# FlowEternal/multitask-hydranet

Hardware: AMD Instinct MI355X
Metric: images/sec (fwd+bwd) HydraNet @ default res, 1/2/4/8 MI355X; CPU-ref same run (higher is better)
Workload: dtype bf16; 1 GPU; full HydraNet (backbone + BiFPN + seg/det/lane heads + multitask loss), big cfg, fwd+loss+bwd; batch_per_gpu=16, global_batch=16, resolution=3x512x1024, parallelism=dp1, hipgraph=True

## Files before the change

include/hydranet_hip.h:

```cpp
#ifndef HYDRANET_HIP_H
#define HYDRANET_HIP_H

#ifdef __cplusplus
extern "C" {
#endif

typedef struct ihipStream_t* hipStream_t;


int hn_gconv_pack_diag(const float* w, void* wk, void* wd, int C, hipStream_t stream);
int hn_pack_weight(const float* w, void* wp, void* wt, int Cout, int Cin, int taps, hipStream_t stream);
int hn_pack_weight_ex(const float* w, void* wp, void* wt, int Cout, int Cin_total, int ci0, int Cin, int taps, int phase, const float* bias,
                      float* b_eff, hipStream_t stream);
int hn_phase_fold(const float* dw_eff, const float* dw1, const float* db_eff, float* dw, float* db, int K, int C0, int C1, hipStream_t stream);
int hn_pack_weights_batched(const long* jobs, int njobs, long total_blocks, const int* block_job, hipStream_t stream);
int hn_pack_small_batched(const long* jobs, const int* block_job, long total_blocks, hipStream_t stream);

int hn_conv_gemm_nt(const void* x0, const void* x1, int mode, int n_img, int H, int W, int C0, int C1, int ld0, int ld1, int up, long M,
                    const void* w, int Nout, int KP, int taps, const float* bias, int act, void* out, int out_f32, int ldc, long rpi,
                    long img_stride, float* psum, float* psq, hipStream_t stream);
int hn_nt_stat_rows(long M, int Nout);
int hn_nt_stat_tile(long M, int Nout);
int hn_conv_gemm_nt_stream(const void* x, int ld0, long M, int C0, const void* w, int Nout, int KP, const float* bias, int act, void* out,
                           int ldc, float* psum, float* psq, int wg_limit, hipStream_t stream);
// ... 6 lines not shown
                        int ldc, const float* coef, int nlev, const long* rows, hipStream_t stream);
int hn_conv_gemm_nt_lvlout(const void* x0, int ld0, long M, int C0, const void* w, int Nout, int KP, const float* bias, int act, float* out,
                           int ldc, long img_stride, int n_img, int nlev, const int* H, const int* W, int row_align, hipStream_t stream);

int hn_conv_gemm_nt_ex(const void* x0, const void* x1, int mode, int n_img, int H, int W, int C0, int C1, int ld0, int ld1, int up, long M,
                       const void* w, int Nout, int KP, int taps, const float* bias, int act, void* out, int out_f32, int ldc, long rpi,
                       long img_stride, float* psum, float* psq, const float* xscale, const float* xshift, const float* xgate, long xhw,
                       int xact, const void* addend, int ld_add, int add_mode, hipStream_t stream);
int hn_conv_gemm_nt_stat(const void* x0, const void* x1, int mode, int n_img, int H, int W, int C0, int C1, int ld0, int ld1, int up, long M,
                         const void* w, int Nout, int KP, int taps, const float* bias, int act, void* out, int out_f32, int ldc, long rpi,
                         long img_stride, float* psum, float* psq, const void* addend, int ld_add, int add_mode, int emode, const void* ez,
                         int ld_ez, const float* ecoef, hipStream_t stream);
int hn_conv_gemm_nt_stat3(const void* x0, int ld0, long M, int C0, const void* w, int Nout, int KP, void* out, int ldc, float* psum, float* psq,
                          const void* addend, int ld_add, const void* ez, int ld_ez, const void* ey, int ld_ey, const float* ecoef,
                          hipStream_t stream);
int hn_wgrad_plan(int mode, int n_img, int H, int W, long M, int Nout, int KP, int taps, int* splits, long* rows_per_split, long* ws_bytes);
int hn_conv_gemm_tn(const void* x0, const void* x1, int mode, int n_img, int H, int W, int C0, int C1, int ld0, int ld1, int up, long M,
                    const void* dz, int ldz, int Nout, int KP, int taps, float* workspace, float* dw, hipStream_t stream);


int hn_stem_fwd(const float* x, const float* w, void* z, void* patches, int N, int H, int W, hipStream_t stream);

int hn_gconv_pack(const float* w, void* wk, void* wd, int C, int flip, hipStream_t stream);
int hn_gconv_fwd(const void* in, int ldi, const void* wk, void* out, int ldo, int N, int Hi, int Wi, int C, int stride, hipStream_t stream);
int hn_gconv_dgrad_s2(const void* dz, int ldz, const void* wd, void* dx, int ldx, int N, int Hi, int Wi, int C, hipStream_t stream);
long hn_wgrad_chunks(long pixels, long items);
int hn_gconv_wgrad(const void* x, int ldx, const void* dz, int ldz, float* part, int N, int Hi, int Wi, int C, int stride,
                   hipStream_t stream);

int hn_dw_pack(const float* w, void* wk, void* wkf, int C, hipStream_t stream);
int hn_dwconv_fwd(const void* in, int ldi, const void* wk, void* out, int ldo, int N, int H, int W, int C, hipStream_t stream);
int hn_dwconv_fwd_levels(const void* in, int ldi, const void* wk, void* out, int ldo, int N, int C, int nlev, const int* H, const int* W,
                         int row_align, int accumulate, hipStream_t stream);
long hn_dwconv_wgrad_blocks(long strips, int C);
int hn_dwconv_wgrad(const void* x, int ldx, const void* dz, int ldz, float* part, int N, int H, int W, int C, hipStream_t stream);
int hn_dwconv_wgrad_levels(const void* x, int ldx, const void* dz, int ldz, float* part, int N, int C, int nlev, const int* H, const int* W,
                           int row_align, hipStream_t stream);
long hn_dwconv_bwd_blocks(long strips, int C);
long hn_dwconv_bwd_blocks_levels(int N, int C, int nlev, const int* H, const int* W);
int hn_dwconv_bwd_levels(const void* dz, int ldz, const void* x, int ldx, const void* wf, void* dx, int lddx, float* part, int N, int C,
                         int nlev, const int* H, const int* W, int row_align, int accumulate, hipStream_t stream);

int hn_maxpool_fwd(const void* in, int ldi, void* out, int ldo, int N, int H, int W, int C, int mode, hipStream_t stream);
int hn_maxpool_bwd(const void* in, int ldi, const void* dout, int ldd, void* dx, int ldx, const float* wscale, int N, int H, int W, int C,
                   int mode, hipStream_t stream);
int hn_maxpool_bwd2(const void* in, int ldi, const void* dout, int ldd, void* dx, int ldx, const float* wscale, void* arg_ws, int N, int H,
                    int W, int C, int mode, int accumulate, hipStream_t stream);

int hn_up2_fwd(const void* in, int ldi, void* out, int ldo, int N, int H, int W, int C, hipStream_t stream);
int hn_sum2x2(const void* g, int ldg, void* out, int ldo, const float* wscale, int N, int H, int W, int C, int accumulate, hipStream_t stream);

int hn_fuse_dweights(const float* pw, int blocks, const float* praw, int nw, float eps, float* dp, hipStream_t stream);
int hn_fuse_fwd(const void* const* in, const int* ld, const int* mode, const float* w, void* out, int ldo, int N, int H, int W, int C,
                hipStream_t stream);
int hn_fuse_fwd_raw(const void* const* in, const int* ld, const int* mode, const float* praw, int nw, float eps, float* wn, void* out, int ldo,
                    int N, int H, int W, int C, hipStream_t stream);
int hn_fuse_bwd_blocks(int N, int H, int W, int C);
int hn_fuse_bwd(const void* const* in, const int* ld, const int* mode, const float* w, const void* dout, int ldd, void* g, int ldg,
                void* const* din, const int* ldin, const int* acc, float* pw, int N, int H, int W, int C, hipStream_t stream);
int hn_fuse_bwd_arg(const void* const* in, const int* ld, const int* mode, const float* w, const void* dout, int ldd, void* g, int ldg,
                    void* const* din, const int* ldin, const int* acc, float* pw, void* const* arg_out, int N, int H, int W, int C,
                    hipStream_t stream);
int hn_maxpool_bwd_from_arg(const void* arg, const void* dout, int ldd, void* dx, int ldx, const float* wscale, int N, int H, int W, int C,
                            int mode, int accumulate, hipStream_t stream);

long hn_fold_ring_rows(int H, int W);
// ... 359 lines not shown
```

multitask_hydranet_amd/csrc/hn_stencil.hip:

```cpp
#include "hn_common.h"

__global__ __launch_bounds__(256) void stem_fwd_kernel(const float* x, const float* w, bf16* z, bf16* patches, int N, int H, int W) {
    const int bidx = xcd_remap(blockIdx.x, gridDim.x);
    __shared__ float sw[27][32];
    for (int i = threadIdx.x; i < 27 * 32; i += 256) {
        const int co = i & 31, t = i >> 5;
        sw[t][co] = w[co * 27 + t];
    }
    __syncthreads();
    const int Ho = H >> 1, Wo = W >> 1, Wp = (Wo + 1) >> 1;
    const long total = (long)N * Ho * Wp;
    const long idx = (long)bidx * 256 + threadIdx.x;
    if (idx >= total) return;
    const int ox = (int)(idx % Wp) * 2;
    const long t1 = idx / Wp;
    const int oy = (int)(t1 % Ho);
    const long n = t1 / Ho;
    const bool two = ox + 1 < Wo;
    float acc[2][32];
#pragma unroll
    for (int c = 0; c < 32; ++c) { acc[0][c] = 0.f; acc[1][c] = 0.f; }
    __shared__ __attribute__((aligned(16))) bf16 sp[2][256][36];
    bf16* prow = patches ? sp[0][threadIdx.x] : nullptr;
    constexpr int PH = 256 * 36;
// ... 830 lines not shown
                    bf16x4 v;
                    if (accumulate) {
                        const bf16x4 prev = ld4(dst);
#pragma unroll
                        for (int k = 0; k < 4; ++k) v[k] = f2bf(da[k] + bf2f(prev[k]));
                    } else {
#pragma unroll
                        for (int k = 0; k < 4; ++k) v[k] = f2bf(da[k]);
                    }
                    *reinterpret_cast<bf16x4*>(dst) = v;
                }
            }
        }
    }
    __syncthreads();
    float* red = reinterpret_cast<float*>(smem);
    if (active) {
#pragma unroll
        for (int tq = 0; tq < 9; ++tq)
#pragma unroll
            for (int k = 0; k < 4; ++k) red[(colh * C4 + cq) * 37 + tq * 4 + k] = acc[tq][k];
    }
    __syncthreads();
    float* dst = part + (long)bidx * C * 9;
    for (int o = tid; o < C4 * 36; o += 256) {
        const int g = o / 36, v = o - g * 36;
        float sum = 0.f;
#pragma unroll
        for (int c2 = 0; c2 < 8; ++c2) sum += red[(c2 * C4 + g) * 37 + v];
        dst[(long)(g * 4 + (v & 3)) * 9 + (v >> 2)] = sum;
    }
}

__global__ void dw_pack_kernel(const float* w, bf16* wk, bf16* wkf, int C) {
    const int idx = blockIdx.x * blockDim.x + threadIdx.x;
    if (idx >= 9 * C) return;
    const int c = idx % C, tap = idx / C;
    const bf16 v = f2bf(w[c * 9 + tap]);
    wk[idx] = v;
    if (wkf) wkf[(8 - tap) * C + c] = v;
}

__device__ __forceinline__ void pool_window(const bf16* in, int ldi, long n, int H, int W, int oy, int ox, int c, int mode, float* best,
                                            int* arg) {
#pragma unroll
    for (int k = 0; k < 8; ++k) { best[k] = -INFINITY; arg[k] = -1; }
    const int off = mode ? -1 : 0;
#pragma unroll
    for (int ky = 0; ky < 3; ++ky)
#pragma unroll
        for (int kx = 0; kx < 3; ++kx) {
            const int iy = 2 * oy + ky + off, ix = 2 * ox + kx + off;
            const bool inside = iy >= 0 && iy < H && ix >= 0 && ix < W;
            if (!inside && mode) continue;
            bf16x8 v = inside ? ld8(in + ((n * H + iy) * (long)W + ix) * ldi + c) : zero8();
#pragma unroll
            for (int k = 0; k < 8; ++k) {
                const float f = bf2f(v[k]);
                if (f > best[k]) { best[k] = f; arg[k] = inside ? ky * 3 + kx : 9; }
            }
        }
}

__global__ __launch_bounds__(256) void maxpool_fwd_kernel(const bf16* in, int ldi, bf16* out, int ldo, int N, int H, int W, int C,
                                                          int mode) {
    const int bidx = xcd_remap(blockIdx.x, gridDim.x);
// ... 284 lines not shown
        const int yq = (int)(t % Hq);
        const long n = t / Hq;
        float qsum[8];
#pragma unroll
        for (int k = 0; k < 8; ++k) qsum[k] = 0.f;
        for (int sub = 0; sub < (quads ? 4 : 1); ++sub) {
        const int x = quads ? 2 * xq + (sub & 1) : xq, y = quads ? 2 * yq + (sub >> 1) : yq;
        float v[3][8], pre[8];
#pragma unroll
        for (int k = 0; k < 8; ++k) pre[k] = 0.f;
#pragma unroll
        for (int i = 0; i < 3; ++i) {
            if (!p.mode[i]) continue;
            if (p.mode[i] == 3 && q.arg[i]) {
                int a[8];
                pool_window(p.in[i], p.ld[i], n, 2 * p.H, 2 * p.W, y, x, cg * 8, 0, v[i], a);
                unsigned long long packed = 0ull;
#pragma unroll
                for (int k = 0; k < 8; ++k) packed |= (unsigned long long)(a[k] & 0xff) << (8 * k);
                *reinterpret_cast<unsigned long long*>(q.arg[i] + ((n * p.H + y) * (long)p.W + x) * p.C + cg * 8) = packed;
            } else {
                fuse_gather(p, i, n, y, x, cg * 8, v[i]);
            }
            const float wi = p.w[i];
#pragma unroll
            for (int k = 0; k < 8; ++k) pre[k] = fmaf(wi, v[i][k], pre[k]);
        }
        const long orow = (n * p.H + y) * (long)p.W + x;
        const bf16x8 d = ld8(q.dout + orow * q.ldd + cg * 8);
        float gg[8];
        bf16x8 go;
#pragma unroll
        for (int k = 0; k < 8; ++k) { gg[k] = bf2f(d[k]) * act_bwd(pre[k], HN_ACT_SWISH); go[k] = f2bf(gg[k]); qsum[k] += bf2f(go[k]); }
        st8(q.g + orow * q.ldg + cg * 8, go);
#pragma unroll
        for (int i = 0; i < 3; ++i) {
            if (!p.mode[i]) continue;
#pragma unroll
            for (int k = 0; k < 8; ++k) dw[i] = fmaf(gg[k], v[i][k], dw[i]);
            if (p.mode[i] == 1 && q.din[i]) {
                const float wi = p.w[i];
                bf16* dst = q.din[i] + orow * q.ldin[i] + cg * 8;
                bf16x8 o;
                if (q.acc[i]) {
                    const bf16x8 prev = ld8(dst);
#pragma unroll
                    for (int k = 0; k < 8; ++k) o[k] = f2bf(fmaf(wi, gg[k], bf2f(prev[k])));
                } else {
#pragma unroll
                    for (int k = 0; k < 8; ++k) o[k] = f2bf(wi * gg[k]);
                }
                st8(dst, o);
            }
        }
        }
        if (quads) {
            const float ws = p.w[up_i];
            bf16* dst = q.din[up_i] + ((n * Hq + yq) * (long)Wq + xq) * q.ldin[up_i] + cg * 8;
            bf16x8 o;
            if (q.acc[up_i]) {
                const bf16x8 prev = ld8(dst);
#pragma unroll
                for (int k = 0; k < 8; ++k) o[k] = f2bf(fmaf(qsum[k], ws, bf2f(prev[k])));
            } else {
#pragma unroll
                for (int k = 0; k < 8; ++k) o[k] = f2bf(qsum[k] * ws);
            }
// ... 35 lines not shown
        const int yq = (int)(t % Hq);
        const long n = t / Hq;
        const long orow0 = (n * p.H + 2 * yq) * (long)p.W + 2 * xq, lrow = (n * Hq + yq) * (long)Wq + xq;
        bf16x8 rd[4], ra[4], rprev[4], rup, rprev_up;
#pragma unroll
        for (int s = 0; s < 4; ++s) rd[s] = ld8(q.dout + (orow0 + (s >> 1) * p.W + (s & 1)) * q.ldd + cg * 8);
#pragma unroll
        for (int s = 0; s < 4; ++s) ra[s] = ld8(ina + (orow0 + (s >> 1) * p.W + (s & 1)) * lda + cg * 8);
        rup = ld8(inb + lrow * ldb + cg * 8);
        if (acca) {
#pragma unroll
            for (int s = 0; s < 4; ++s) rprev[s] = ld8(da + (orow0 + (s >> 1) * p.W + (s & 1)) * ldda + cg * 8);
        }
        bf16* dup = db + lrow * lddb + cg * 8;
        if (accb) rprev_up = ld8(dup);
        float qsum[8], vb[8];
#pragma unroll
        for (int k = 0; k < 8; ++k) { qsum[k] = 0.f; vb[k] = bf2f(rup[k]); }
#pragma unroll
        for (int s = 0; s < 4; ++s) {
            const long orow = orow0 + (s >> 1) * p.W + (s & 1);
            float gg[8];
            bf16x8 go;
#pragma unroll
            for (int k = 0; k < 8; ++k) {
                const float va = bf2f(ra[s][k]);
                const float pre = a_first ? fmaf(wb, vb[k], fmaf(wa, va, 0.f)) : fmaf(wa, va, fmaf(wb, vb[k], 0.f));
                gg[k] = bf2f(rd[s][k]) * act_bwd(pre, HN_ACT_SWISH);
                go[k] = f2bf(gg[k]);
                qsum[k] += bf2f(go[k]);
                dwa = fmaf(gg[k], va, dwa);
                dwb = fmaf(gg[k], vb[k], dwb);
            }
            st8(q.g + orow * q.ldg + cg * 8, go);
            if (da) {
                bf16x8 o;
                if (acca) {
#pragma unroll
                    for (int k = 0; k < 8; ++k) o[k] = f2bf(fmaf(wa, gg[k], bf2f(rprev[s][k])));
                } else {
#pragma unroll
                    for (int k = 0; k < 8; ++k) o[k] = f2bf(wa * gg[k]);
                }
                st8(da + orow * ldda + cg * 8, o);
            }
        }
        bf16x8 o;
        if (accb) {
#pragma unroll
            for (int k = 0; k < 8; ++k) o[k] = f2bf(fmaf(qsum[k], wb, bf2f(rprev_up[k])));
        } else {
#pragma unroll
            for (int k = 0; k < 8; ++k) o[k] = f2bf(qsum[k] * wb);
        }
        st8(dup, o);
    }
    __shared__ float red[4][3];
    const int lane = threadIdx.x & 63, wave = threadIdx.x >> 6;
    float dw[3] = {0.f, 0.f, 0.f};
#pragma unroll
    for (int i = 0; i < 3; ++i) dw[i] = i == ia ? dwa : (i == ib ? dwb : 0.f);
#pragma unroll
    for (int i = 0; i < 3; ++i) {
        const float sm = wave_sum(dw[i]);
        if (lane == 0) red[wave][i] = sm;
    }
    __syncthreads();
// ... 241 lines not shown
    HN_CHECK_ARG(x && dz && part && (C & 7) == 0 && C <= 2048 && ((ldx | ldz) & 7) == 0);
    L.work_off[0] = 0;
    for (int l = 0; l < L.n; ++l) L.work_off[l + 1] = L.work_off[l] + (long)N * L.H[l] * ((L.W[l] + 3) >> 2);
    const long strips = L.work_off[L.n];
    const int lanes = 256 / (C >> 3);
    const long blocks = hn_dwconv_wgrad_blocks(strips, C);
    const int spl = (int)((strips + blocks * lanes - 1) / (blocks * lanes));
    hipLaunchKernelGGL(dwconv_wgrad_kernel, dim3(blocks), dim3(256), 0, st, (const bf16*)x, ldx, (const bf16*)dz, ldz, part, N, C, spl, L);
    HN_LAUNCH_CHECK();
}
extern "C" int hn_dwconv_wgrad(const void* x, int ldx, const void* dz, int ldz, float* part, int N, int H, int W, int C, hipStream_t st) {
    Levels L;
    const int rc = fill_levels(L, N, 1, &H, &W);
    return rc != HN_OK ? rc : dwconv_wgrad_launch(x, ldx, dz, ldz, part, N, C, L, st);
}
extern "C" int hn_dwconv_wgrad_levels(const void* x, int ldx, const void* dz, int ldz, float* part, int N, int C, int nlev, const int* H,
                                      const int* W, int row_align, hipStream_t st) {
    Levels L;
    const int rc = fill_levels(L, N, nlev, H, W, row_align);
    return rc != HN_OK ? rc : dwconv_wgrad_launch(x, ldx, dz, ldz, part, N, C, L, st);
}

static long dwconv_bwd_strip_blocks(long strips, int C) {
    const int lanes = 256 / (C >> 2);
    const long tb = g_hn_knob[7] > 0 ? g_hn_knob[7] : 768;
    long spl = (strips + (tb - 1) * lanes) / (tb * lanes);
    if (spl < 2) spl = 2;
    return (strips + spl * lanes - 1) / (spl * lanes);
}
extern "C" long hn_dwconv_bwd_blocks(long strips, int C) { return dwconv_bwd_strip_blocks(strips, C); }
static size_t dwconv_bwd_tiled_lds(int C8) {
    return (size_t)((((DWT_TH + 2) * 18 * C8 + 63) >> 6) + ((DWT_TH * 16 * C8 + 63) >> 6)) * 1024;
}
static bool dwconv_bwd_tiled_plan(int N, int C, const Levels& L, DwTiles& T, int& tpw, long& blocks) {
    T.tile_off[0] = 0;
    for (int l = 0; l < L.n; ++l) {
        T.ty[l] = (L.H[l] + DWT_TH - 1) / DWT_TH;
        T.tx[l] = (L.W[l] + 15) >> 4;
        T.tile_off[l + 1] = T.tile_off[l] + (long)N * T.ty[l] * T.tx[l];
    }
    const long total = T.tile_off[L.n];
    const int C8 = C >> 3;
    const size_t lds = dwconv_bwd_tiled_lds(C8);
#ifdef HN_NO_DW_TILED
    return false;
#endif
    if (g_hn_knob[7] < 0 || C8 > 16 || lds > 80 * 1024 || total < 512) return false;
    tpw = (int)((total + 511) / 512);
    blocks = (total + tpw - 1) / tpw;
    return true;
}
extern "C" long hn_dwconv_bwd_blocks_levels(int N, int C, int nlev, const int* H, const int* W) {
    Levels L;
    if (fill_levels(L, N, nlev, H, W) != HN_OK || (C & 7) || C < 8) return -1;
    DwTiles T;
    int tpw = 0;
    long blocks = 0;
    if (dwconv_bwd_tiled_plan(N, C, L, T, tpw, blocks)) return blocks;
    long strips = 0;
    for (int l = 0; l < nlev; ++l) strips += (long)N * H[l] * ((W[l] + 3) >> 2);
    return dwconv_bwd_strip_blocks(strips, C);
}
extern "C" int hn_dwconv_bwd_levels(const void* dz, int ldz, const void* x, int ldx, const void* wf, void* dx, int lddx, float* part, int N, int C,
                                    int nlev, const int* H, const int* W, int row_align, int accumulate, hipStream_t st) {
    Levels L;
    const int rc = fill_levels(L, N, nlev, H, W, row_align);
    if (rc != HN_OK) return rc;
    HN_CHECK_ARG(dz && x && part && (!dx || wf) && (C & 7) == 0 && C >= 8 && C <= 1024 && ((ldz | ldx) & 7) == 0 && (!dx || (lddx & 7) == 0));
    long pad_items = 0;
    if (dx && !accumulate)
        for (int l = 0; l < L.n; ++l) pad_items += (L.row_off[l + 1] - L.row_off[l] - (long)N * L.H[l] * L.W[l]) * (C >> 3);
    DwTiles T;
    int tpw = 0;
    long tblocks = 0;
    if (dwconv_bwd_tiled_plan(N, C, L, T, tpw, tblocks)) {
        const int C8 = C >> 3;
        const size_t lds = dwconv_bwd_tiled_lds(C8);
        if (lds > 64 * 1024) {
            static std::atomic<unsigned long long> optin_t{0};
            if (!lds_optin(optin_t, {(const void*)dwconv_bwd_tiled_kernel<true>, (const void*)dwconv_bwd_tiled_kernel<false>})) return HN_ERR_LAUNCH;
        }
        L.work_off[0] = 0;
        if (dx)
            hipLaunchKernelGGL(dwconv_bwd_tiled_kernel<true>, dim3((unsigned)(tblocks + cdiv(pad_items, 256))), dim3(256), lds, st, (const bf16*)dz,
                               ldz, (const bf16*)x, ldx, (const bf16*)wf, (bf16*)dx, lddx, part, N, C, tpw, (int)tblocks, L, T, accumulate);
        else
            hipLaunchKernelGGL(dwconv_bwd_tiled_kernel<false>, dim3((unsigned)tblocks), dim3(256), lds, st, (const bf16*)dz, ldz, (const bf16*)x, ldx,
                               (const bf16*)wf, (bf16*)dx, lddx, part, N, C, tpw, (int)tblocks, L, T, accumulate);
        HN_LAUNCH_CHECK();
    }
    L.work_off[0] = 0;
    for (int l = 0; l < L.n; ++l) L.work_off[l + 1] = L.work_off[l] + (long)N * L.H[l] * ((L.W[l] + 3) >> 2);
    const long strips = L.work_off[L.n];
    const int lanes = 256 / (C >> 2);
    const long blocks = dwconv_bwd_strip_blocks(strips, C);
    const int spl = (int)((strips + blocks * lanes - 1) / (blocks * lanes));
    const size_t lds = (256 * 37 + 9 * (size_t)C) * sizeof(float);
    if (lds > 64 * 1024) {
        static std::atomic<unsigned long long> optin{0};
        if (!lds_optin(optin, {(const void*)dwconv_bwd_kernel})) return HN_ERR_LAUNCH;
    }
    hipLaunchKernelGGL(dwconv_bwd_kernel, dim3((unsigned)(blocks + cdiv(pad_items, 256))), dim3(256), lds, st, (const bf16*)dz, ldz, (const bf16*)x,
                       ldx, (const bf16*)wf, (bf16*)dx, lddx, part, N, C, spl, blocks, L, accumulate);
    HN_LAUNCH_CHECK();
}

extern "C" int hn_maxpool_fwd(const void* in, int ldi, void* out, int ldo, int N, int H, int W, int C, int mode, hipStream_t st) {
    HN_CHECK_ARG(in && out && (C & 7) == 0 && ((ldi | ldo) & 7) == 0 && !(H & 1) && !(W & 1) && (mode == 0 || mode == 1));
    hipLaunchKernelGGL(maxpool_fwd_kernel, dim3(ew_grid((long)N * (H >> 1) * (W >> 1) * (C >> 3))), dim3(256), 0, st, (const bf16*)in, ldi,
                       (bf16*)out, ldo, N, H, W, C, mode);
    HN_LAUNCH_CHECK();
}
extern "C" int hn_maxpool_bwd(const void* in, int ldi, const void* dout, int ldd, void* dx, int ldx, const float* wscale, int N, int H,
                              int W, int C, int mode, hipStream_t st) {
    HN_CHECK_ARG(in && dout && dx && (C & 7) == 0 && ((ldi | ldd | ldx) & 7) == 0 && !(H & 1) && !(W & 1));
    hipLaunchKernelGGL(maxpool_bwd_kernel, dim3(ew_grid((long)N * H * W * (C >> 3))), dim3(256), 0, st, (const bf16*)in, ldi,
                       (const bf16*)dout, ldd, (bf16*)dx, ldx, wscale, N, H, W, C, mode);
    HN_LAUNCH_CHECK();
}
extern "C" int hn_maxpool_bwd2(const void* in, int ldi, const void* dout, int ldd, void* dx, int ldx, const float* wscale, void* arg_ws,
                               int N, int H, int W, int C, int mode, int accumulate, hipStream_t st) {
    HN_CHECK_ARG(in && dout && dx && arg_ws && (C & 7) == 0 && ((ldi | ldd | ldx) & 7) == 0 && !(H & 1) && !(W & 1));
    hipLaunchKernelGGL(maxpool_arg_kernel, dim3(ew_grid((long)N * (H >> 1) * (W >> 1) * (C >> 3))), dim3(256), 0, st, (const bf16*)in, ldi,
                       (unsigned char*)arg_ws, N, H, W, C, mode);
    hipLaunchKernelGGL(maxpool_bwd_arg_kernel, dim3(ew_grid((long)N * H * W * (C >> 3))), dim3(256), 0, st, (const unsigned char*)arg_ws,
                       (const bf16*)dout, ldd, (bf16*)dx, ldx, wscale, N, H, W, C, mode, accumulate);
    HN_LAUNCH_CHECK();
}
extern "C" int hn_maxpool_bwd_from_arg(const void* arg, const void* dout, int ldd, void* dx, int ldx, const float* wscale, int N, int H, int W,
                                       int C, int mode, int accumulate, hipStream_t st) {
    HN_CHECK_ARG(arg && dout && dx && (C & 7) == 0 && ((ldd | ldx) & 7) == 0 && !(H & 1) && !(W & 1));
    hipLaunchKernelGGL(maxpool_bwd_arg_kernel, dim3(ew_grid((long)N * H * W * (C >> 3))), dim3(256), 0, st, (const unsigned char*)arg,
                       (const bf16*)dout, ldd, (bf16*)dx, ldx, wscale, N, H, W, C, mode, accumulate);
    HN_LAUNCH_CHECK();
}
extern "C" int hn_up2_fwd(const void* in, int ldi, void* out, int ldo, int N, int H, int W, int C, hipStream_t st) {
    HN_CHECK_ARG(in && out && (C & 7) == 0 && ((ldi | ldo) & 7) == 0);
    hipLaunchKernelGGL(up2_fwd_kernel, dim3(ew_grid((long)N * 4 * H * W * (C >> 3))), dim3(256), 0, st, (const bf16*)in, ldi, (bf16*)out, ldo,
                       N, H, W, C);
// ... 13 lines not shown
    for (int i = 0; i < 3; ++i) {
        f.in[i] = (const bf16*)in[i]; f.ld[i] = ld[i]; f.mode[i] = mode[i];
        HN_CHECK_ARG(mode[i] >= 0 && mode[i] <= 3 && (mode[i] == 0 || (in[i] && (ld[i] & 7) == 0)));
        HN_CHECK_ARG(mode[i] != 2 || (!(H & 1) && !(W & 1)));
    }
    f.w = w; f.out = (bf16*)out; f.ldo = ldo; f.N = N; f.H = H; f.W = W; f.C = C;
    f.praw = nullptr; f.nw = 0; f.eps = 0.f; f.wn = nullptr;
    return HN_OK;
}
extern "C" int hn_fuse_fwd(const void* const* in, const int* ld, const int* mode, const float* w, void* out, int ldo, int N, int H, int W,
                           int C, hipStream_t st) {
    Fuse f;
    HN_CHECK_ARG(out);
    const int rc = fill_fuse(f, in, ld, mode, w, out, ldo, N, H, W, C);
    if (rc) return rc;
    hipLaunchKernelGGL(fuse_fwd_kernel, dim3(ew_grid((long)N * H * W * (C >> 3))), dim3(256), 0, st, f);
    HN_LAUNCH_CHECK();
}
extern "C" int hn_fuse_fwd_raw(const void* const* in, const int* ld, const int* mode, const float* praw, int nw, float eps, float* wn,
                               void* out, int ldo, int N, int H, int W, int C, hipStream_t st) {
    Fuse f;
    HN_CHECK_ARG(out && praw && wn && nw >= 1 && nw <= 3);
    const int rc = fill_fuse(f, in, ld, mode, nullptr, out, ldo, N, H, W, C);
    if (rc) return rc;
    f.praw = praw; f.nw = nw; f.eps = eps; f.wn = wn;
    hipLaunchKernelGGL(fuse_fwd_kernel, dim3(ew_grid((long)N * H * W * (C >> 3))), dim3(256), 0, st, f);
    HN_LAUNCH_CHECK();
}
extern "C" int hn_fuse_bwd_blocks(int N, int H, int W, int C) {
    long b = ((long)N * H * W * (C >> 3) + 255) / 256;
    if (b > 1024) b = 1024;
    return (int)(b < 1 ? 1 : b);
}
extern "C" int hn_fuse_bwd(const void* const* in, const int* ld, const int* mode, const float* w, const void* dout, int ldd, void* g,
                           int ldg, void* const* din, const int* ldin, const int* acc, float* pw, int N, int H, int W, int C,
                           hipStream_t st) {
    FuseBwd q;
    HN_CHECK_ARG(dout && g && pw && din && ldin && ((ldd | ldg) & 7) == 0);
    const int rc = fill_fuse(q.f, in, ld, mode, w, nullptr, 8, N, H, W, C);
    if (rc) return rc;
    q.dout = (const bf16*)dout; q.ldd = ldd; q.g = (bf16*)g; q.ldg = ldg; q.pw = pw;
    for (int i = 0; i < 3; ++i) { q.din[i] = (bf16*)din[i]; q.ldin[i] = ldin[i]; q.acc[i] = acc ? acc[i] : 0; q.arg[i] = nullptr; }
    int n_id = 0, n_up = 0, n_pool = 0, up_dst = 0;
    for (int i = 0; i < 3; ++i) { n_id += mode[i] == 1; n_up += mode[i] == 2; n_pool += mode[i] == 3; up_dst += mode[i] == 2 && q.din[i]; }
    if (n_id == 1 && n_up == 1 && up_dst == 1 && n_pool == 0 && !(H & 1) && !(W & 1))
        hipLaunchKernelGGL(fuse_bwd_quads_kernel, dim3(hn_fuse_bwd_blocks(N, H, W, C)), dim3(256), 0, st, q);
    else
        hipLaunchKernelGGL(fuse_bwd_kernel, dim3(hn_fuse_bwd_blocks(N, H, W, C)), dim3(256), 0, st, q);
    HN_LAUNCH_CHECK();
}
extern "C" int hn_fuse_bwd_arg(const void* const* in, const int* ld, const int* mode, const float* w, const void* dout, int ldd, void* g,
                               int ldg, void* const* din, const int* ldin, const int* acc, float* pw, void* const* arg_out, int N, int H,
                               int W, int C, hipStream_t st) {
    FuseBwd q;
    HN_CHECK_ARG(dout && g && pw && din && ldin && arg_out && ((ldd | ldg) & 7) == 0);
    const int rc = fill_fuse(q.f, in, ld, mode, w, nullptr, 8, N, H, W, C);
    if (rc) return rc;
    q.dout = (const bf16*)dout; q.ldd = ldd; q.g = (bf16*)g; q.ldg = ldg; q.pw = pw;
    for (int i = 0; i < 3; ++i) {
        q.din[i] = (bf16*)din[i]; q.ldin[i] = ldin[i]; q.acc[i] = acc ? acc[i] : 0;
        q.arg[i] = mode[i] == 3 ? (unsigned char*)arg_out[i] : nullptr;
    }
    int n_id = 0, n_up = 0, n_pool = 0, up_dst = 0;
    for (int i = 0; i < 3; ++i) { n_id += mode[i] == 1; n_up += mode[i] == 2; n_pool += mode[i] == 3; up_dst += mode[i] == 2 && q.din[i]; }
    if (n_id == 1 && n_up == 1 && up_dst == 1 && n_pool == 0 && !(H & 1) && !(W & 1))
        hipLaunchKernelGGL(fuse_bwd_quads_kernel, dim3(hn_fuse_bwd_blocks(N, H, W, C)), dim3(256), 0, st, q);
    else
        hipLaunchKernelGGL(fuse_bwd_kernel, dim3(hn_fuse_bwd_blocks(N, H, W, C)), dim3(256), 0, st, q);
    HN_LAUNCH_CHECK();
}

extern "C" int hn_seg_fold(const void* dvp, int ldv, int c0, void* out, int ldo, const void* yprev, int ldy, int N, int H, int W, int C,
                           int up, hipStream_t st) {
    HN_CHECK_ARG(dvp && out && (C & 7) == 0 && (c0 & 7) == 0 && ((ldv | ldo) & 7) == 0 && H >= 4 && W >= 4 && up >= 0 && up <= 2);
    HN_CHECK_ARG(!yprev || (ldy & 7) == 0);
    const int clamp = up == 2;
    if (clamp) up = 0;
    hipLaunchKernelGGL(seg_fold_kernel, dim3(ew_grid((long)N * (H >> up) * (W >> up) * (C >> 3))), dim3(256), 0, st, (const bf16*)dvp, ldv, c0,
                       (bf16*)out, ldo, (const bf16*)yprev, ldy, N, H, W, C, up, clamp);
    HN_LAUNCH_CHECK();
}

extern "C" int hn_space_to_depth(const float* dy, void* out, int ldo, int N, int h, int w, int k, hipStream_t st) {
    HN_CHECK_ARG(dy && out && N > 0 && h > 0 && w > 0 && k > 0 && ldo >= 4 * k && (ldo & 7) == 0);
    hipLaunchKernelGGL(space_to_depth_kernel, dim3(ew_grid((long)N * h * w * ldo)), dim3(256), 0, st, dy, (bf16*)out, ldo, N, h, w, k);
    HN_LAUNCH_CHECK();
}

extern "C" int hn_space_to_depth_blocks(int N, int h, int w, int k) { return ew_grid((long)N * h * w * 4 * (k >> 3)); }
extern "C" int hn_space_to_depth_bf16(const void* in, int ldi, void* out, int N, int h, int w, int k, float* psum, hipStream_t st) {
// ... 93 lines not shown
```

multitask_hydranet_amd/ops/heads.py:

```python
from __future__ import annotations

import ctypes
import os
from typing import Optional, Sequence, Tuple

import torch

from .._lib import lib, policy
from .core import *
from .backbone import *
from .neck import *
from .seg import *


class HeadOut(torch.autograd.Function):

    @staticmethod
    def forward(ctx, dw_weight, pw_weight, bias, k, act, *feats):
        n = feats[0].shape[0]
        cout, cin = pw_weight.shape[0], pw_weight.shape[1]
        wp, wt = pack_conv_weight(pw_weight)
        rows_total = sum(f.shape[1] * f.shape[2] for f in feats)
        rep = cout // k
        out = torch.empty((n, rows_total * rep, k), device=feats[0].device, dtype=F32)
# ... 113 lines not shown
        d6 = new_act(n, h // 2, w // 2, c, dout.device)
        lib().call("hn_sum2x2", ptr(dout[..., 3 * c:]), ld(dout), ptr(d6), ld(d6), None, n, h // 2, w // 2, c, 0)
        return d3, d4, d5, d6



def packed_rows(geom):
    n, hs, ws = geom
    return sum(_pad_rows(n * h * w) for h, w in zip(hs, ws))


def has_pad_rows(geom):
    n, hs, ws = geom
    return any((n * h * w) % LEVEL_ALIGN for h, w in zip(hs, ws))


def _ptr_array(tensors):
    return (ctypes.c_void_p * len(tensors))(*[t.data_ptr() if t is not None else None for t in tensors])


def level_views(packed, geom):
    n, hs, ws = geom
    out, off = [], 0
    for h, w in zip(hs, ws):
        m = n * h * w
        out.append(packed[0, 0, off:off + m].view(n, h, w, packed.shape[3]))
        off += _pad_rows(m)
    return out


def k_dwconv_levels(x, wk, geom, into=None):
    nl, H, W, _, _ = _geom_arrays(geom)
    out = torch.empty_like(x) if into is None else into
    lib().call("hn_dwconv_fwd_levels", ptr(x), ld(x), ptr(wk), ptr(out), ld(out), geom[0], x.shape[3], nl, ctypes.addressof(H),
               ctypes.addressof(W), LEVEL_ALIGN, 0 if into is None else 1)
    return out


def k_dwconv_wgrad_levels(x, dz, geom):
    nl, H, W, _, _ = _geom_arrays(geom)
    c = x.shape[3]
    chunks = lib().query("hn_dwconv_wgrad_blocks", sum(geom[0] * hh * ((ww + 3) // 4) for hh, ww in zip(geom[1], geom[2])), c)
    part = torch.empty((chunks, c * 9), device=x.device, dtype=F32)
    lib().call("hn_dwconv_wgrad_levels", ptr(x), ld(x), ptr(dz), ld(dz), ptr(part), geom[0], c, nl, ctypes.addressof(H), ctypes.addressof(W),
               LEVEL_ALIGN)
    return k_rows_reduce(part, 1, chunks, c * 9).view(c, 1, 3, 3)


class PackLevels(torch.autograd.Function):

    @staticmethod
    def forward(ctx, *feats):
        n, c = feats[0].shape[0], feats[0].shape[3]
        geom = (n, tuple(f.shape[1] for f in feats), tuple(f.shape[2] for f in feats))
        total = packed_rows(geom)
        out = torch.empty((1, 1, total, c), device=feats[0].device, dtype=BF16)
        if PACK_LEVELS_ONE and all(f.stride(3) == 1 and f.stride(1) == f.shape[2] * f.stride(2) and f.stride(0) == f.shape[1] * f.stride(1)
                                   for f in feats):
            nl, H, W, _, _ = _geom_arrays(geom)
            lds = (ctypes.c_int * nl)(*[ld(f) for f in feats])
            srcs = _ptr_array(feats)
            lib().call("hn_pack_levels", ctypes.addressof(srcs), ctypes.addressof(lds), ptr(out), ld(out), n, c, nl,
                       ctypes.addressof(H), ctypes.addressof(W), LEVEL_ALIGN)
        else:
            for v, f in zip(level_views(out, geom), feats):
                k_eltwise(2, f, alpha=1.0, out=v)
# ... 174 lines not shown
```

multitask_hydranet_amd/ops/neck.py:

```python
from __future__ import annotations

import ctypes
import os
from typing import Optional, Sequence, Tuple

import torch

from .._lib import lib, policy
from .core import *
from .backbone import *


def k_dwconv(x, wk, out=None):
    n, h, w, c = x.shape
    if out is None:
        out = new_act(n, h, w, c, x.device)
    lib().call("hn_dwconv_fwd", ptr(x), ld(x), ptr(wk), ptr(out), ld(out), n, h, w, c)
    return out


def k_dwconv_wgrad(x, dz):
    n, h, w, c = x.shape
    chunks = lib().query("hn_dwconv_wgrad_blocks", n * h * ((w + 3) // 4), c)
    part = torch.empty((chunks, c * 9), device=x.device, dtype=F32)
    lib().call("hn_dwconv_wgrad", ptr(x), ld(x), ptr(dz), ld(dz), ptr(part), n, h, w, c)
    return k_rows_reduce(part, 1, chunks, c * 9).view(c, 1, 3, 3)


def k_dwconv_bwd(dz, x, wf, geom=None, want_dx=True, into=None, queue=None, weight=None):
    c = x.shape[3]
    if geom is None:
        n, h, w, _ = x.shape
        H, W, nl, align = (ctypes.c_int * 1)(h), (ctypes.c_int * 1)(w), 1, 1
    else:
        nl, H, W, _, _ = _geom_arrays(geom)
        n, align = geom[0], LEVEL_ALIGN
    blocks = lib().query("hn_dwconv_bwd_blocks_levels", n, c, nl, ctypes.addressof(H), ctypes.addressof(W))
    part = torch.empty((blocks, c * 9), device=x.device, dtype=F32)
    dx = None
    if want_dx:
        dx = torch.empty_like(dz) if into is None else into
    lib().call("hn_dwconv_bwd_levels", ptr(dz), ld(dz), ptr(x), ld(x), ptr(wf), ptr(dx), ld(dx) if dx is not None else 0, ptr(part), n, c, nl,
               ctypes.addressof(H), ctypes.addressof(W), align, 0 if into is None else 1)
    if queue is not None:
        queue.add_rows(weight, part, blocks, c * 9, (c, 1, 3, 3))
        return dx, None
    return dx, k_rows_reduce(part, 1, blocks, c * 9).view(c, 1, 3, 3)


# ... 93 lines not shown

class Fuse(torch.autograd.Function):

    @staticmethod
    def forward(ctx, praw, m0, m1, m2, a, b, c, slots=None):
        ins = [a, b, c]
        modes = [m0, m1, m2]
        n, h, wd, ch = a.shape
        assert m0 == 1
        dev = a.device
        w = torch.empty((3,), device=dev, dtype=F32)
        out = new_act(n, h, wd, ch, dev)
        ap, al, am = _fuse_args(ins, modes)
        lib().call("hn_fuse_fwd_raw", ctypes.addressof(ap), ctypes.addressof(al), ctypes.addressof(am), ptr(praw), praw.numel(), 1e-4, ptr(w),
                   ptr(out), ld(out), n, h, wd, ch)
        ctx.modes = modes
        ctx.slots = slots if slots is not None else (None, None, None)
        ctx.queue, ctx.pref = (cur_queue() if praw.requires_grad else None), praw
        ctx.save_for_backward(praw, w, *[t for t in ins if t is not None])
        return out

    @staticmethod
    def backward(ctx, dout):
        praw, w = ctx.saved_tensors[0], ctx.saved_tensors[1]
        rest = list(ctx.saved_tensors[2:])
        ins = [rest.pop(0) if m else None for m in ctx.modes]
        dpraw, dins = fuse_backward(praw, w, ins, ctx.modes, ctx.slots, ctx.queue, ctx.pref, dense(dout))
        return dpraw, None, None, None, dins[0], dins[1], dins[2], None


def fuse_backward(praw, w, ins, modes, slots, queue, pref, dout):
    n, h, wd, ch = dout.shape
    dev = dout.device
    g = new_act(n, h, wd, ch, dev)
    dst, accum = [None] * 3, [0] * 3
    for i, m in enumerate(modes):
        if not m:
            continue
        sl = slots[i]
        if sl is not None and sl.buf is not None:
            dst[i], accum[i] = sl.buf, 1
        else:
            dst[i] = new_act(*ins[i].shape, dev)
            if sl is not None:
                sl.buf = dst[i]
    ap, al, am = _fuse_args(ins, modes)
    inside = (1, 2) if FUSE_SUM2X2 else (1,)
    dp_ = (ctypes.c_void_p * 3)(*[ptr(dst[i]) if modes[i] in inside else None for i in range(3)])
    dl = (ctypes.c_int * 3)(*[ld(dst[i]) if modes[i] in inside else 0 for i in range(3)])
    da = (ctypes.c_int * 3)(*accum)
    blocks = lib().query("hn_fuse_bwd_blocks", n, h, wd, ch)
    pw = torch.empty((blocks, 3), device=dev, dtype=F32)
    args = [torch.empty((n * h * wd * ch,), device=dev, dtype=torch.uint8) if (m == 3 and FUSE_ARG) else None for m in modes]
    aa = (ctypes.c_void_p * 3)(*[ptr(t) for t in args])
    lib().call("hn_fuse_bwd_arg", ctypes.addressof(ap), ctypes.addressof(al), ctypes.addressof(am), ptr(w), ptr(dout), ld(dout), ptr(g),
               ld(g), ctypes.addressof(dp_), ctypes.addressof(dl), ctypes.addressof(da), ptr(pw), ctypes.addressof(aa), n, h, wd, ch)
    if queue is not None:
        dpraw = queue.add_fuse(pref, pw, blocks, 1e-4)
    else:
        dpraw = torch.empty_like(praw)
        lib().call("hn_fuse_dweights", ptr(pw), blocks, ptr(praw), praw.numel(), 1e-4, ptr(dpraw))
    for i, m in enumerate(modes):
        if m == 2 and not FUSE_SUM2X2:
            lib().call("hn_sum2x2", ptr(g), ld(g), ptr(dst[i]), ld(dst[i]), ptr(w[i]), n, h // 2, wd // 2, ch, accum[i])
        elif m == 3 and not FUSE_ARG:
            k_maxpool_bwd(ins[i], g, 0, wscale=w[i], into=dst[i], accumulate=bool(accum[i]))
        elif m == 3:
            lib().call("hn_maxpool_bwd_from_arg", ptr(args[i]), ptr(g), ld(g), ptr(dst[i]), ld(dst[i]), ptr(w[i]), n, 2 * h, 2 * wd, ch, 0,
                       accum[i])
    return dpraw, [None if (slots[i] is not None or not modes[i]) else dst[i] for i in range(3)]


__all__ = [n for n in dir() if not n.startswith("__")]
```

Measured before the change: 991.6 images/sec.

## Add LDS-tiled depthwise conv forward and skip unread fuse-bwd gradient buffer

Adds a tiled depthwise 3x3 forward kernel. It stages an (8+2)x18 pixel halo tile into LDS with async global-to-LDS loads, then sweeps rows with a rolling 3-row register window. Channel counts up to 128 on large inputs are routed to it by default, aiming to cut redundant global reads compared with the per-pixel kernel. Separately, fuse backward no longer allocates or writes the intermediate gradient tensor g when no pooling or unfused upsample consumer reads it, which saves a full activation write. The cost is more dispatch logic and extra grid blocks for zeroing padding rows.

```diff
diff --git a/include/hydranet_hip.h b/include/hydranet_hip.h
--- a/include/hydranet_hip.h
+++ b/include/hydranet_hip.h
@@ -62,6 +62,9 @@
 int hn_dwconv_fwd(const void* in, int ldi, const void* wk, void* out, int ldo, int N, int H, int W, int C, hipStream_t stream);
 int hn_dwconv_fwd_levels(const void* in, int ldi, const void* wk, void* out, int ldo, int N, int C, int nlev, const int* H, const int* W,
                          int row_align, int accumulate, hipStream_t stream);
+int hn_dwconv_fwd_levels_tiled(const void* in, int ldi, const void* wk, void* out, int ldo, int N, int C, int nlev, const int* H, const int* W,
+                               int row_align, int accumulate, int wg_limit, hipStream_t stream);
+int hn_dwconv_fwd_tiled_ok(int N, int C, int nlev, const int* H, const int* W);
 long hn_dwconv_wgrad_blocks(long strips, int C);
 int hn_dwconv_wgrad(const void* x, int ldx, const void* dz, int ldz, float* part, int N, int H, int W, int C, hipStream_t stream);
 int hn_dwconv_wgrad_levels(const void* x, int ldx, const void* dz, int ldz, float* part, int N, int C, int nlev, const int* H, const int* W,
diff --git a/multitask_hydranet_amd/csrc/hn_stencil.hip b/multitask_hydranet_amd/csrc/hn_stencil.hip
--- a/multitask_hydranet_amd/csrc/hn_stencil.hip
+++ b/multitask_hydranet_amd/csrc/hn_stencil.hip
@@ -886,6 +886,102 @@
     }
 }
 
+__global__ __launch_bounds__(256, 4) void dwconv_fwd_tiled_kernel(const bf16* in, int ldi, const bf16* wk, bf16* out, int ldo, int N, int C, int tpw,
+                                                                  int blocks, const Levels L, const DwTiles T) {
+    extern __shared__ __attribute__((aligned(16))) char smem[];
+    constexpr int TH = DWT_TH, ZPX = (TH + 2) * 18;
+    const int C8 = C >> 3, C4 = C >> 2;
+    const int tid = threadIdx.x, lane = tid & 63, wave = __builtin_amdgcn_readfirstlane(tid >> 6);
+    if ((int)blockIdx.x >= blocks) {
+        long idx = ((long)blockIdx.x - blocks) * 256 + tid;
+        for (int l = 0; l < L.n; ++l) {
+            const long real = (long)N * L.H[l] * L.W[l];
+            const long pad = L.row_off[l + 1] - L.row_off[l] - real;
+            if (idx < pad * C8) {
+                st8(out + (L.row_off[l] + real + idx / C8) * ldo + (idx % C8) * 8, zero8());
+                return;
+            }
+            idx -= pad * C8;
+        }
+        return;
+    }
+    const int ZCH = (ZPX * C8 + 63) >> 6;
+    const int bidx = xcd_remap(blockIdx.x, blocks);
+    const long total = T.tile_off[L.n];
+    const long t0 = (long)bidx * tpw;
+    long t1 = t0 + tpw;
+    if (t1 > total) t1 = total;
+    const int cstep = C4 <= 16 ? 16 : 8;
+    const int cq = tid % C4, colh = tid / C4;
+    const bool active = colh < cstep;
+    float wr[9][4];
+#pragma unroll
+    for (int tq = 0; tq < 9; ++tq) {
+        const bf16x4 wv = active ? ld4(wk + tq * C + cq * 4) : zero4();
+#pragma unroll
+        for (int k = 0; k < 4; ++k) wr[tq][k] = bf2f(wv[k]);
+    }
+    const unsigned magic = (65536u + C8 - 1) / C8;
+    int lv = 0;
+    for (long t = t0; t < t1; ++t) {
+        while (lv + 1 < L.n && t >= T.tile_off[lv + 1]) ++lv;
+        const int H = L.H[lv], W = L.W[lv];
+        long lt = t - T.tile_off[lv];
+        const int tx = (int)(lt % T.tx[lv]);
+        lt /= T.tx[lv];
+        const int ty = (int)(lt % T.ty[lv]);
+        const long n = lt / T.ty[lv];
+        const int oy0 = ty * TH, ox0 = tx * 16;
+        const long row0 = L.row_off[lv] + n * H * (long)W;
+        __syncthreads();
+        for (int ch = wave; ch < ZCH; ch += 4) {
+            const int e = ch * 64 + lane;
+            const int px = (int)(((unsigned)e * magic) >> 16), pc = e - px * C8;
+            const int py = px / 18, pxx = px - py * 18;
+            const int iy = oy0 - 1 + py, ix = ox0 - 1 + pxx;
+            const bf16* src = (px < ZPX && iy >= 0 && iy < H && ix >= 0 && ix < W) ? in + (row0 + (long)iy * W + ix) * ldi + pc * 8 : st_zero_piece;
+            st_glds16(src, smem + ch * 1024);
+        }
+        asm volatile("s_waitcnt vmcnt(0)" ::: "memory");
+        __syncthreads();
+        if (active)
+#pragma unroll 1
+        for (int col = colh; col < 16; col += cstep) {
+            float win[3][3][4];
+            auto load_row = [&](int py, float (&w3)[3][4]) {
+#pragma unroll
+                for (int j = 0; j < 3; ++j) {
+                    const bf16x4 v = *reinterpret_cast<const bf16x4*>(smem + ((py * 18 + col + j) * C4 + cq) * 8);
+#pragma unroll
+                    for (int k = 0; k < 4; ++k) w3[j][k] = bf2f(v[k]);
+                }
+            };
+            load_row(0, win[0]);
+            load_row(1, win[1]);
+#pragma unroll
+            for (int r = 0; r < TH; ++r) {
+                load_row(r + 2, win[(r + 2) % 3]);
+                float acc[4] = {0.f, 0.f, 0.f, 0.f};
+#pragma unroll
+                for (int rr = 0; rr < 3; ++rr) {
+                    const int iy = oy0 + r - 1 + rr;
+                    if (iy < 0 || iy >= H) continue;
+#pragma unroll
+                    for (int j = 0; j < 3; ++j)
+#pragma unroll
+                        for (int k = 0; k < 4; ++k) acc[k] = fmaf(win[(r + rr) % 3][j][k], wr[rr * 3 + j][k], acc[k]);
+                }
+                if (oy0 + r < H && ox0 + col < W) {
+                    bf16x4 v;
+#pragma unroll
+                    for (int k = 0; k < 4; ++k) v[k] = f2bf(acc[k]);
+                    *reinterpret_cast<bf16x4*>(out + (row0 + (long)(oy0 + r) * W + ox0 + col) * ldo + cq * 4) = v;
+                }
+            }
+        }
+    }
+}
+
 __global__ void dw_pack_kernel(const float* w, bf16* wk, bf16* wkf, int C) {
     const int idx = blockIdx.x * blockDim.x + threadIdx.x;
     if (idx >= 9 * C) return;
@@ -1236,7 +1332,7 @@
         bf16x8 go;
 #pragma unroll
         for (int k = 0; k < 8; ++k) { gg[k] = bf2f(d[k]) * act_bwd(pre[k], HN_ACT_SWISH); go[k] = f2bf(gg[k]); qsum[k] += bf2f(go[k]); }
-        st8(q.g + orow * q.ldg + cg * 8, go);
+        if (q.g) st8(q.g + orow * q.ldg + cg * 8, go);
 #pragma unroll
         for (int i = 0; i < 3; ++i) {
             if (!p.mode[i]) continue;
@@ -1338,7 +1434,7 @@
                 dwa = fmaf(gg[k], va, dwa);
                 dwb = fmaf(gg[k], vb[k], dwb);
             }
-            st8(q.g + orow * q.ldg + cg * 8, go);
+            if (q.g) st8(q.g + orow * q.ldg + cg * 8, go);
             if (da) {
                 bf16x8 o;
                 if (acca) {
@@ -1646,14 +1742,17 @@
 static size_t dwconv_bwd_tiled_lds(int C8) {
     return (size_t)((((DWT_TH + 2) * 18 * C8 + 63) >> 6) + ((DWT_TH * 16 * C8 + 63) >> 6)) * 1024;
 }
-static bool dwconv_bwd_tiled_plan(int N, int C, const Levels& L, DwTiles& T, int& tpw, long& blocks) {
+static long dwconv_tiles(int N, const Levels& L, DwTiles& T) {
     T.tile_off[0] = 0;
     for (int l = 0; l < L.n; ++l) {
         T.ty[l] = (L.H[l] + DWT_TH - 1) / DWT_TH;
         T.tx[l] = (L.W[l] + 15) >> 4;
         T.tile_off[l + 1] = T.tile_off[l] + (long)N * T.ty[l] * T.tx[l];
     }
-    const long total = T.tile_off[L.n];
+    return T.tile_off[L.n];
+}
+static bool dwconv_bwd_tiled_plan(int N, int C, const Levels& L, DwTiles& T, int& tpw, long& blocks) {
+    const long total = dwconv_tiles(N, L, T);
     const int C8 = C >> 3;
     const size_t lds = dwconv_bwd_tiled_lds(C8);
 #ifdef HN_NO_DW_TILED
@@ -1719,6 +1818,42 @@
     HN_LAUNCH_CHECK();
 }
 
+#define DWF_MAX_C 128
+#define DWF_MAX_TILES (1L << 30)
+extern "C" int hn_dwconv_fwd_tiled_ok(int N, int C, int nlev, const int* H, const int* W) {
+    if (N <= 0 || C < 8 || (C & 7) || C > DWF_MAX_C || nlev < 1 || nlev > HN_MAX_LEVELS || !H || !W) return 0;
+    long tiles = 0;
+    for (int l = 0; l < nlev; ++l) {
+        if (H[l] <= 0 || W[l] <= 0) return 0;
+        tiles += (long)N * ((H[l] + DWT_TH - 1) / DWT_TH) * ((W[l] + 15) >> 4);
+        if (tiles > DWF_MAX_TILES) return 0;
+    }
+    return 1;
+}
+extern "C" int hn_dwconv_fwd_levels_tiled(const void* in, int ldi, const void* wk, void* out, int ldo, int N, int C, int nlev, const int* H,
+                                          const int* W, int row_align, int accumulate, int wg_limit, hipStream_t st) {
+    HN_CHECK_ARG(in && wk && out && wg_limit >= 0 && (accumulate == 0 || accumulate == 1));
+    Levels L;
+    const int rc = fill_levels(L, N, nlev, H, W, row_align);
+    if (rc != HN_OK) return rc;
+    const auto a16 = [](const void* q) { return (reinterpret_cast<uintptr_t>(q) & 15) == 0; };
+    if (!hn_dwconv_fwd_tiled_ok(N, C, nlev, H, W) || accumulate || (ldi & 7) || (ldo & 7) || ldi < C || ldo < C || !a16(in) || !a16(wk) || !a16(out))
+        return HN_ERR_UNSUPPORTED;
+    DwTiles T;
+    const long total = dwconv_tiles(N, L, T);
+    const long blocks = wg_limit > 0 ? wg_limit : total;
+    const int tpw = (int)((total + blocks - 1) / blocks);
+    long pad_items = 0;
+    for (int l = 0; l < L.n; ++l) pad_items += (L.row_off[l + 1] - L.row_off[l] - (long)N * L.H[l] * L.W[l]) * (C >> 3);
+    const long grid = blocks + cdiv(pad_items, 256);
+    if (grid > 0x7fffffffL) return HN_ERR_UNSUPPORTED;
+    const size_t lds = (size_t)(((DWT_TH + 2) * 18 * (C >> 3) + 63) >> 6) * 1024;
+    L.work_off[0] = 0;
+    hipLaunchKernelGGL(dwconv_fwd_tiled_kernel, dim3((unsigned)grid), dim3(256), lds, st, (const bf16*)in, ldi, (const bf16*)wk, (bf16*)out, ldo, N, C,
+                       tpw, (int)blocks, L, T);
+    HN_LAUNCH_CHECK();
+}
+
 extern "C" int hn_maxpool_fwd(const void* in, int ldi, void* out, int ldo, int N, int H, int W, int C, int mode, hipStream_t st) {
     HN_CHECK_ARG(in && out && (C & 7) == 0 && ((ldi | ldo) & 7) == 0 && !(H & 1) && !(W & 1) && (mode == 0 || mode == 1));
     hipLaunchKernelGGL(maxpool_fwd_kernel, dim3(ew_grid((long)N * (H >> 1) * (W >> 1) * (C >> 3))), dim3(256), 0, st, (const bf16*)in, ldi,
@@ -1798,13 +1933,19 @@
     if (b > 1024) b = 1024;
     return (int)(b < 1 ? 1 : b);
 }
+static bool fuse_bwd_g_unread(const int* mode, void* const* din) {
+    for (int i = 0; i < 3; ++i)
+        if (mode[i] == 3 || (mode[i] == 2 && !din[i])) return false;
+    return true;
+}
 extern "C" int hn_fuse_bwd(const void* const* in, const int* ld, const int* mode, const float* w, const void* dout, int ldd, void* g,
                            int ldg, void* const* din, const int* ldin, const int* acc, float* pw, int N, int H, int W, int C,
                            hipStream_t st) {
     FuseBwd q;
-    HN_CHECK_ARG(dout && g && pw && din && ldin && ((ldd | ldg) & 7) == 0);
+    HN_CHECK_ARG(dout && pw && din && ldin && ((ldd | (g ? ldg : 0)) & 7) == 0);
     const int rc = fill_fuse(q.f, in, ld, mode, w, nullptr, 8, N, H, W, C);
     if (rc) return rc;
+    HN_CHECK_ARG(g || fuse_bwd_g_unread(mode, din));
     q.dout = (const bf16*)dout; q.ldd = ldd; q.g = (bf16*)g; q.ldg = ldg; q.pw = pw;
     for (int i = 0; i < 3; ++i) { q.din[i] = (bf16*)din[i]; q.ldin[i] = ldin[i]; q.acc[i] = acc ? acc[i] : 0; q.arg[i] = nullptr; }
     int n_id = 0, n_up = 0, n_pool = 0, up_dst = 0;
@@ -1819,9 +1960,10 @@
                                int ldg, void* const* din, const int* ldin, const int* acc, float* pw, void* const* arg_out, int N, int H,
                                int W, int C, hipStream_t st) {
     FuseBwd q;
-    HN_CHECK_ARG(dout && g && pw && din && ldin && arg_out && ((ldd | ldg) & 7) == 0);
+    HN_CHECK_ARG(dout && pw && din && ldin && arg_out && ((ldd | (g ? ldg : 0)) & 7) == 0);
     const int rc = fill_fuse(q.f, in, ld, mode, w, nullptr, 8, N, H, W, C);
     if (rc) return rc;
+    HN_CHECK_ARG(g || fuse_bwd_g_unread(mode, din));
     q.dout = (const bf16*)dout; q.ldd = ldd; q.g = (bf16*)g; q.ldg = ldg; q.pw = pw;
     for (int i = 0; i < 3; ++i) {
         q.din[i] = (bf16*)din[i]; q.ldin[i] = ldin[i]; q.acc[i] = acc ? acc[i] : 0;
diff --git a/multitask_hydranet_amd/ops/heads.py b/multitask_hydranet_amd/ops/heads.py
--- a/multitask_hydranet_amd/ops/heads.py
+++ b/multitask_hydranet_amd/ops/heads.py
@@ -169,6 +169,10 @@
 def k_dwconv_levels(x, wk, geom, into=None):
     nl, H, W, _, _ = _geom_arrays(geom)
     out = torch.empty_like(x) if into is None else into
+    if into is None and dw_fwd_tiled_route(x, wk, out, geom[0], x.shape[3], geom[1], geom[2]):
+        lib().call("hn_dwconv_fwd_levels_tiled", ptr(x), ld(x), ptr(wk), ptr(out), ld(out), geom[0], x.shape[3], nl, ctypes.addressof(H),
+                   ctypes.addressof(W), LEVEL_ALIGN, 0, 0)
+        return out
     lib().call("hn_dwconv_fwd_levels", ptr(x), ld(x), ptr(wk), ptr(out), ld(out), geom[0], x.shape[3], nl, ctypes.addressof(H),
                ctypes.addressof(W), LEVEL_ALIGN, 0 if into is None else 1)
     return out
diff --git a/multitask_hydranet_amd/ops/neck.py b/multitask_hydranet_amd/ops/neck.py
--- a/multitask_hydranet_amd/ops/neck.py
+++ b/multitask_hydranet_amd/ops/neck.py
@@ -11,10 +11,36 @@
 from .backbone import *
 
 
+DW_FWD_TILED = policy("HN_DW_FWD_TILED", "1") != "0"
+DW_FWD_TILED_MAX_C = 128
+DW_FWD_TILED_MAX_TILES = 1 << 30
+DW_FWD_TILED_MIN_TILES = 1024
+
+
+def dw_fwd_tiles(n: int, hs: Sequence[int], ws: Sequence[int]) -> int:
+    return sum(n * ((h + 7) // 8) * ((w + 15) // 16) for h, w in zip(hs, ws))
+
+
+def dw_fwd_tiled_ok(n: int, c: int, hs: Sequence[int], ws: Sequence[int]) -> bool:
+    return (n > 0 and 8 <= c <= DW_FWD_TILED_MAX_C and c % 8 == 0 and 1 <= len(hs) <= 5 and len(hs) == len(ws)
+            and all(h > 0 and w > 0 for h, w in zip(hs, ws)) and dw_fwd_tiles(n, hs, ws) <= DW_FWD_TILED_MAX_TILES)
+
+
+def dw_fwd_tiled_route(x, wk, out, n, c, hs, ws) -> bool:
+    if not DW_FWD_TILED or not dw_fwd_tiled_ok(n, c, hs, ws) or dw_fwd_tiles(n, hs, ws) < DW_FWD_TILED_MIN_TILES:
+        return False
+    return (ld(x) % 8 == 0 and ld(out) % 8 == 0 and ld(x) >= c and ld(out) >= c and x.data_ptr() % 16 == 0 and out.data_ptr() % 16 == 0
+            and wk.data_ptr() % 16 == 0)
+
+
 def k_dwconv(x, wk, out=None):
     n, h, w, c = x.shape
     if out is None:
         out = new_act(n, h, w, c, x.device)
+    if dw_fwd_tiled_route(x, wk, out, n, c, (h,), (w,)):
+        H, W = (ctypes.c_int * 1)(h), (ctypes.c_int * 1)(w)
+        lib().call("hn_dwconv_fwd_levels_tiled", ptr(x), ld(x), ptr(wk), ptr(out), ld(out), n, c, 1, ctypes.addressof(H), ctypes.addressof(W), 1, 0, 0)
+        return out
     lib().call("hn_dwconv_fwd", ptr(x), ld(x), ptr(wk), ptr(out), ld(out), n, h, w, c)
     return out
 
@@ -174,7 +200,8 @@
 def fuse_backward(praw, w, ins, modes, slots, queue, pref, dout):
     n, h, wd, ch = dout.shape
     dev = dout.device
-    g = new_act(n, h, wd, ch, dev)
+    g_read = any(m == 3 or (m == 2 and not FUSE_SUM2X2) for m in modes)
+    g = new_act(n, h, wd, ch, dev) if g_read else None
     dst, accum = [None] * 3, [0] * 3
     for i, m in enumerate(modes):
         if not m:
@@ -196,7 +223,7 @@
     args = [torch.empty((n * h * wd * ch,), device=dev, dtype=torch.uint8) if (m == 3 and FUSE_ARG) else None for m in modes]
     aa = (ctypes.c_void_p * 3)(*[ptr(t) for t in args])
     lib().call("hn_fuse_bwd_arg", ctypes.addressof(ap), ctypes.addressof(al), ctypes.addressof(am), ptr(w), ptr(dout), ld(dout), ptr(g),
-               ld(g), ctypes.addressof(dp_), ctypes.addressof(dl), ctypes.addressof(da), ptr(pw), ctypes.addressof(aa), n, h, wd, ch)
+               ld(g) if g is not None else 0, ctypes.addressof(dp_), ctypes.addressof(dl), ctypes.addressof(da), ptr(pw), ctypes.addressof(aa), n, h, wd, ch)
     if queue is not None:
         dpraw = queue.add_fuse(pref, pw, blocks, 1e-4)
     else:
```

Result: no change. 993.6 images/sec (median of 6 runs) (+0.2%).
